# succinctlabs/kzg-rs

Hardware: NVIDIA B200
Metric: blobs verified/sec (verify_blob_kzg_proof_batch) (higher is better)
Workload: dtype u32-limb modular integer (Fr 255-bit / Fp 381-bit) + SHA-256

## Files before the change

### include/kzgb200.h

```cpp
#ifndef KZGB200_H
#define KZGB200_H
#include <stddef.h>
#include <stdint.h>
#ifdef __cplusplus
extern "C" {
#endif

#define KZGB200_OK 0
#define KZGB200_BAD_ARGS 1
#define KZGB200_INTERNAL_ERROR 2
#define KZGB200_INVALID_LENGTH 3
#define KZGB200_INVALID_SETUP 5

#define KZGB200_BYTES_PER_BLOB 131072
#define KZGB200_BYTES_PER_COMMITMENT 48
#define KZGB200_BYTES_PER_PROOF 48
#define KZGB200_BYTES_PER_FIELD_ELEMENT 32
#define KZGB200_PARTIAL_BYTES 352

typedef struct kzgb200_ctx kzgb200_ctx;

int kzgb200_create(kzgb200_ctx** out, int device, const uint8_t* g2_points, size_t g2_points_len);
void kzgb200_destroy(kzgb200_ctx* ctx);
const char* kzgb200_last_error(const kzgb200_ctx* ctx);

int kzgb200_verify_kzg_proof(kzgb200_ctx* ctx, const uint8_t* commitment48, const uint8_t* z32, const uint8_t* y32,
                             const uint8_t* proof48, int* ok);

int kzgb200_verify_blob_kzg_proof(kzgb200_ctx* ctx, const uint8_t* blob, const uint8_t* commitment48,
                                  const uint8_t* proof48, int* ok, uint8_t* z_out, uint8_t* y_out);

int kzgb200_verify_blob_kzg_proof_batch(kzgb200_ctx* ctx, const uint8_t* blobs, size_t n_blobs,
                                        const uint8_t* commitments, size_t n_commitments,
                                        const uint8_t* proofs, size_t n_proofs, int* ok,
                                        uint8_t* z_out, uint8_t* y_out);
int kzgb200_verify_blob_kzg_proof_batch_device(kzgb200_ctx* ctx, const uint8_t* d_blobs, const uint8_t* d_commitments,
                                               const uint8_t* d_proofs, size_t n, int* ok,
                                               uint8_t* d_z_out, uint8_t* d_y_out);

int kzgb200_verify_kzg_proof_many(kzgb200_ctx* ctx, const uint8_t* commitments, const uint8_t* zs, const uint8_t* ys,
                                  const uint8_t* proofs, size_t m, uint8_t* verdicts);

int kzgb200_verify_kzg_proof_batch(kzgb200_ctx* ctx, const uint8_t* commitments104, const uint8_t* zs32, const uint8_t* ys32,
                                   const uint8_t* proofs104, size_t n, int* ok);

int kzgb200_verify_blob_kzg_proof_batch_each(kzgb200_ctx* ctx, const uint8_t* blobs, const uint8_t* commitments, const uint8_t* proofs,
                                             size_t n, uint8_t* verdicts, uint8_t* z_out, uint8_t* y_out);

int kzgb200_compute_challenge(kzgb200_ctx* ctx, const uint8_t* blob, const uint8_t* commitment48, uint8_t* z_out32);
int kzgb200_evaluate_polynomial_in_evaluation_form(kzgb200_ctx* ctx, const uint8_t* blob, const uint8_t* z32, uint8_t* y_out32);

typedef struct kzgb200_group kzgb200_group;
int kzgb200_group_create(kzgb200_group** out, const int* device_ids, int n_devices, const uint8_t* g2_points, size_t g2_points_len,
                         size_t max_blobs_per_device);
int kzgb200_group_join(kzgb200_group** out, const char* session, int rank, int world, int device, const uint8_t* g2_points,
                       size_t g2_points_len, size_t max_blobs_per_rank);
void kzgb200_group_destroy(kzgb200_group* g);
int kzgb200_group_size(const kzgb200_group* g);
int kzgb200_group_local_members(const kzgb200_group* g);
kzgb200_ctx* kzgb200_group_context(kzgb200_group* g, int local_index);
const char* kzgb200_group_last_error(const kzgb200_group* g);
int kzgb200_group_uses_peer_stores(const kzgb200_group* g, int local_index);
int kzgb200_group_verify_blob_kzg_proof_batch(kzgb200_group* g, const uint8_t* blobs, size_t n_blobs, const uint8_t* commitments,
                                              size_t n_commitments, const uint8_t* proofs, size_t n_proofs, int* ok, uint8_t* z_out,
                                              uint8_t* y_out);
int kzgb200_group_verify_shards(kzgb200_group* g, const uint8_t* const* blobs, const uint8_t* const* commitments,
                                const uint8_t* const* proofs, const size_t* n_local, int device_pointers, int* ok,
                                uint8_t* const* z_out, uint8_t* const* y_out);
int kzgb200_group_last_partials(kzgb200_group* g, uint8_t* out, size_t n_ranks);
int kzgb200_group_host_protocol_test(const char* session, int rank, int world, const uint8_t* commitments, const uint8_t* zy,
                                     const uint8_t* proofs, size_t n_local, size_t chunk, uint8_t* digest_out32);

#define KZGB200_TRANSCRIPT_EXACT 0
#define KZGB200_TRANSCRIPT_TREE 1
#define KZGB200_TRANSCRIPT_EXACT_DEVICE 2
int kzgb200_set_transcript_mode(kzgb200_ctx* ctx, int mode);
int kzgb200_last_r(kzgb200_ctx* ctx, uint8_t* r_out32);
int kzgb200_host_sha256(const uint8_t* msg, size_t len, uint8_t* out32, int force_portable);

int kzgb200_last_partial(kzgb200_ctx* ctx, uint8_t* out352);

int kzgb200_harness_generate(kzgb200_ctx* ctx, uint64_t seed, size_t n, int degree, const uint8_t* tau_powers48,
                             uint8_t* d_blobs, uint8_t* d_commitments, uint8_t* d_proofs);
int kzgb200_load_g1_lagrange(kzgb200_ctx* ctx, const uint8_t* g1_lagrange, size_t n_points);
int kzgb200_blob_to_kzg_commitment_batch(kzgb200_ctx* ctx, const uint8_t* d_blobs, size_t n, uint8_t* d_commitments_out);
int kzgb200_compute_blob_kzg_proof_batch(kzgb200_ctx* ctx, const uint8_t* d_blobs, const uint8_t* d_commitments, size_t n,
                                         uint8_t* d_proofs_out);

int kzgb200_load_cell_setup(kzgb200_ctx* ctx, const uint8_t* g1_monomial48, size_t n_points, const uint8_t* g2_tau64_96);
int kzgb200_verify_cell_kzg_proof_batch(kzgb200_ctx* ctx, const uint8_t* commitments, const uint64_t* cell_indices, const uint8_t* cells,
                                        const uint8_t* proofs, size_t n, int* ok);
int kzgb200_verify_cell_kzg_proof_batch_device(kzgb200_ctx* ctx, const uint8_t* d_commitments, const uint64_t* d_cell_indices,
                                               const uint8_t* d_cells, const uint8_t* d_proofs, size_t n, int* ok);
int kzgb200_compute_cells(kzgb200_ctx* ctx, const uint8_t* blob, uint8_t* cells_out);
int kzgb200_compute_cells_batch_device(kzgb200_ctx* ctx, const uint8_t* d_blobs, size_t n, uint8_t* d_cells);
int kzgb200_harness_generate_cells(kzgb200_ctx* ctx, uint64_t seed, size_t n_blobs, int degree, const uint8_t* tau_powers48,
                                   uint8_t* d_cells, uint8_t* d_commitments, uint8_t* d_proofs);

int kzgb200_set_profiling(kzgb200_ctx* ctx, int on);
int kzgb200_set_slab_tail(kzgb200_ctx* ctx, int on);
int kzgb200_get_phase_ms(kzgb200_ctx* ctx, float* out8);
int kzgb200_debug_final_ticks(kzgb200_ctx* ctx, long long* out14);
int kzgb200_debug_engine_selftest(kzgb200_ctx* ctx, uint32_t seed, int rounds, uint32_t* mismatches32, int* n_programs);
void* kzgb200_stream(kzgb200_ctx* ctx);

typedef struct kzgb200_pipeline kzgb200_pipeline;
int kzgb200_pipeline_create(kzgb200_pipeline** out, int device, const uint8_t* g2_points, size_t g2_points_len, int depth);
void kzgb200_pipeline_destroy(kzgb200_pipeline* p);
int kzgb200_pipeline_depth(const kzgb200_pipeline* p);
kzgb200_ctx* kzgb200_pipeline_context(kzgb200_pipeline* p, int slot);
int kzgb200_pipeline_submit(kzgb200_pipeline* p, const uint8_t* blobs, size_t n_blobs, const uint8_t* commitments,
                            size_t n_commitments, const uint8_t* proofs, size_t n_proofs, uint8_t* z_out, uint8_t* y_out,
                            uint64_t* ticket);
int kzgb200_pipeline_submit_device(kzgb200_pipeline* p, const uint8_t* d_blobs, const uint8_t* d_commitments,
                                   const uint8_t* d_proofs, size_t n, uint8_t* d_z_out, uint8_t* d_y_out, uint64_t* ticket);
int kzgb200_pipeline_wait(kzgb200_pipeline* p, uint64_t ticket, int* ok);

void* kzgb200_alloc_pinned(size_t bytes);
void kzgb200_free_pinned(void* p);

#ifdef __cplusplus
}
#endif
#endif
```

### kzg_rs_b200/csrc/common.cuh

```cuda
#pragma once
#include <cuda_runtime.h>
#include "sha256.cuh"
#include "verify.cuh"
#include "vliw.cuh"
#include "vliw29.cuh"
#include "glv.cuh"

namespace kzgb200 {

constexpr int kFieldElementsPerBlob = 4096;
constexpr int kBytesPerBlob = 4096 * 32;
constexpr uint32_t kErrBlob = 1, kErrCommitment = 2, kErrProof = 4, kErrScalar = 8;
struct ZY { Fr z, y; };

struct DeviceTables {
    Fr twiddle[2048];
    Fr twiddle_po[128][32];
    PairingTables pairing;
    vliw29::LineCoeffs29 lines29[2][kMillerSteps];
    G1Affine gen_table[64][15];
    uint32_t setup_ok;
};

#ifndef KSHA_THREADS
// ... 32 lines not shown
}
__device__ __forceinline__ Fr ldg_fr(const Fr* p) {
    const uint4* q = reinterpret_cast<const uint4*>(p);
    uint4 a = __ldg(q), b = __ldg(q + 1);
    Fr f;
    f.l[0] = a.x; f.l[1] = a.y; f.l[2] = a.z; f.l[3] = a.w; f.l[4] = b.x; f.l[5] = b.y; f.l[6] = b.z; f.l[7] = b.w;
    return f;
}

struct Partial {
    G1 a, b;
    Fr ry;
    uint32_t err;
    uint32_t pad[7];
};

struct FinalSmem {
    G1 sm[kFinalThreads];
    unsigned char pad[20 * 1024];
};
struct PairSmem {
    f29::F29 regs[vliw29::kTotalRegs];
    vliw29::SharedTables stab;
};
struct FinalPts { G1Affine pts[2]; uint32_t go; };

constexpr int kManyStride = vliw::kTotalRegsThr * 12 + 1;
constexpr int kManySmemBytes = kManyGroups * kManyStride * 4 + (int)sizeof(vliw::SharedTables) + vliw::kNumSharedRegs * (int)sizeof(Fp) +
                               kManyGroups * (2 * (int)sizeof(G1Affine) + 2) + 64;
struct CellTables {
    Fr w4096[2048], w4096_inv[2048];
    Fr coset[4096];
    Fr shift64[kCellsPerExtBlob];
    Fr shift_inv[kCellsPerExtBlob];
    Fr w64_inv[kFieldElementsPerCell / 2];
    Fr omega8192, inv64;
    G1Affine tau_tab[kFieldElementsPerCell][4];
    LineCoeffs tau64_lines[kMillerSteps];
    vliw29::LineCoeffs29 lines29[kMillerSteps];
    uint32_t ok;
};
__global__ void setup_tables_kernel(DeviceTables* T, const uint8_t* g2_points);
__global__ void setup_lines29_kernel(DeviceTables* T);
constexpr int kChallengeSlabs = 8;
void launch_challenge(int stages, cudaStream_t st, const uint8_t* blobs, const uint8_t* commitments, int n, Fr* z_mont, ZY* zy, Fr* zpow,
                      const uint8_t* slab_flags = nullptr);
__global__ void eval_kernel(const uint8_t* __restrict__ blobs, int n, const Fr* __restrict__ zpow, const DeviceTables* __restrict__ T,
                            ZY* __restrict__ zy, uint32_t* __restrict__ status);
__global__ void g1_decompress_kernel(const uint8_t* __restrict__ commitments, const uint8_t* __restrict__ proofs, int n, G1Affine* __restrict__ C,
                                     G1Affine* __restrict__ P, uint32_t* __restrict__ status, bool with_subgroup_check);
__global__ void g1_subgroup_kernel(const G1Affine* __restrict__ C, const G1Affine* __restrict__ P, int n, uint32_t* __restrict__ status);
__global__ void transcript_schedule_kernel(const uint8_t* __restrict__ commitments, const ZY* __restrict__ zy, const uint8_t* __restrict__ proofs,
                                           uint64_t n, uint32_t* __restrict__ wk, uint64_t first_blk, uint64_t blk_count);
__global__ void transcript_chain_kernel(const uint32_t* __restrict__ wk_all, uint64_t n, Fr* __restrict__ r_mont, uint32_t* __restrict__ state,
                                        uint64_t first_blk, uint64_t blk_count);
__global__ void transcript_words_kernel(const uint8_t* __restrict__ commitments, const ZY* __restrict__ zy, const uint8_t* __restrict__ proofs,
                                        uint64_t first_entry, uint64_t entry_count, uint32_t* __restrict__ words);
__global__ void transcript_tree_leaf_words_kernel(const uint32_t* __restrict__ words, uint64_t n, uint32_t* __restrict__ digests,
                                                  uint64_t first_group, uint64_t group_count);
__global__ void r_from_digest_kernel(const uint32_t* __restrict__ digest, Fr* __restrict__ r_mont);
__global__ void z_setup_kernel(const uint8_t* __restrict__ z_be32, int n, Fr* __restrict__ z_mont, ZY* __restrict__ zy, Fr* __restrict__ zpow,
                               uint32_t* __restrict__ status);
__global__ void import_parsed_kernel(const uint8_t* __restrict__ c104, const uint8_t* __restrict__ p104, const uint8_t* __restrict__ z32,
                                     const uint8_t* __restrict__ y32, int n, G1Affine* __restrict__ C, G1Affine* __restrict__ P,
                                     uint8_t* __restrict__ c48, uint8_t* __restrict__ p48, Fr* __restrict__ z_mont, ZY* __restrict__ zy);
__global__ void msm_scalars_kernel(const Fr* __restrict__ z_mont, const ZY* __restrict__ zy, const Fr* __restrict__ r_mont, uint64_t offset, int n,
                                   uint8_t* __restrict__ digits, Fr* __restrict__ ry);
__global__ void msm_sort_kernel(const uint8_t* __restrict__ digits, int n, uint32_t* __restrict__ order, uint32_t* __restrict__ start);
void launch_msm_bucket(int ctas_per_sm, int n, int slice, cudaStream_t st, const G1Affine* C, const G1Affine* P, const uint32_t* order,
                       const uint32_t* start, G1* halfsum, G1* part);
void launch_msm_bucket_join(int lanes, int n, int slice, cudaStream_t st, const uint32_t* start, const G1* halfsum, const G1* part, G1* buckets);
__global__ void msm_window_kernel(const G1* __restrict__ buckets, G1* __restrict__ windows);
__global__ void msm_combine_kernel(const G1* __restrict__ windows, const Fr* __restrict__ ry, const uint32_t* __restrict__ status, int n,
                                   const DeviceTables* __restrict__ T, Partial* __restrict__ out, uint32_t* flag, uint32_t epoch);
__global__ void wait_flags_kernel(const uint32_t* flags, int count, uint32_t epoch, uint32_t* __restrict__ timed_out);
__global__ void batch_final_kernel(const Partial* __restrict__ parts, int nparts, const DeviceTables* __restrict__ T, uint32_t* __restrict__ result,
                                   FinalPts* __restrict__ out);
__global__ void single_final_kernel(const G1Affine* __restrict__ C, const G1Affine* __restrict__ P, const ZY* __restrict__ zy,
                                    const uint32_t* __restrict__ status, const DeviceTables* __restrict__ T, uint32_t* __restrict__ result,
                                    FinalPts* __restrict__ out);
__global__ void pairing_check_kernel(const FinalPts* __restrict__ in, const DeviceTables* __restrict__ T, const vliw29::LineCoeffs29* __restrict__ lines_b,
                                     uint32_t* __restrict__ result, long long* __restrict__ ticks);
__global__ void engine_selftest_kernel(uint32_t seed, int rounds, f29::F29* __restrict__ ref, uint32_t* __restrict__ mismatches);
inline void launch_batch_final(cudaStream_t st, const Partial* parts, int nparts, const DeviceTables* T, uint32_t* result, unsigned char* scratch512,
                               bool ticks, const vliw29::LineCoeffs29* lines_b = nullptr) {
    FinalPts* fp = reinterpret_cast<FinalPts*>(scratch512 + 256);
    batch_final_kernel<<<1, kFinalThreads, sizeof(FinalSmem), st>>>(parts, nparts, T, result, fp);
    pairing_check_kernel<<<1, kPairThreads, sizeof(PairSmem), st>>>(fp, T, lines_b, result, ticks ? reinterpret_cast<long long*>(scratch512 + 128) : nullptr);
}
__global__ void many_lhs_kernel(const uint8_t* __restrict__ z32, const uint8_t* __restrict__ y32, const G1Affine* __restrict__ C,
                                const G1Affine* __restrict__ P, size_t m, const DeviceTables* __restrict__ T, G1Affine* __restrict__ X,
                                uint32_t* __restrict__ status);
__global__ void many_lhs_zy_kernel(const ZY* __restrict__ zy, const G1Affine* __restrict__ C, const G1Affine* __restrict__ P, size_t m,
                                   const DeviceTables* __restrict__ T, G1Affine* __restrict__ X, const uint32_t* __restrict__ status);
__global__ void many_pairing_kernel(const G1Affine* __restrict__ X, const G1Affine* __restrict__ P, const uint32_t* __restrict__ status, size_t m,
                                    const DeviceTables* __restrict__ T, uint8_t* __restrict__ verdicts);
__global__ void many_pairing_warp_kernel(const G1Affine* __restrict__ X, const G1Affine* __restrict__ P, size_t m, const DeviceTables* __restrict__ T,
                                         uint8_t* __restrict__ verdicts);
__global__ void export_scalars_kernel(const ZY* __restrict__ zy, int n, uint8_t* __restrict__ z_out, uint8_t* __restrict__ y_out);
__global__ void r_to_raw_kernel(const Fr* __restrict__ r_mont, ZY* __restrict__ out);
__global__ void status_or_kernel(const uint32_t* __restrict__ status, int n, uint32_t* __restrict__ out);
__global__ void harness_parse_points_kernel(const uint8_t* bytes, int n, G1Affine* out, uint32_t* bad);
__global__ void harness_blob_kernel(uint64_t seed, int n, int D, const DeviceTables* __restrict__ T, uint8_t* __restrict__ blobs);
__global__ void harness_commit_kernel(uint64_t seed, int n, int D, const G1Affine* __restrict__ M, const Fr* __restrict__ z_mont,
                                      uint8_t* __restrict__ out, int want_proof);
__global__ void lag_parse_kernel(const uint8_t* __restrict__ bytes, G1Affine* __restrict__ out, uint32_t* __restrict__ bad);
__global__ void lag_table_kernel(const G1Affine* __restrict__ L, G1* __restrict__ table);
__global__ void blob_scalars_kernel(const uint8_t* __restrict__ blobs, int n, Fr* __restrict__ scalars, uint32_t* __restrict__ status);
__global__ void quotient_kernel(const uint8_t* __restrict__ blobs, int n, const Fr* __restrict__ z_mont, const ZY* __restrict__ zy,
                                const DeviceTables* __restrict__ T, Fr* __restrict__ scalars);
__global__ void lag_msm_kernel(const Fr* __restrict__ scalars, int n, const G1* __restrict__ table, uint8_t* __restrict__ out48);
__global__ void cell_setup_kernel(CellTables* T, const uint8_t* __restrict__ g2_tau64);
__global__ void cell_setup_points_kernel(CellTables* T, const uint8_t* __restrict__ g1_monomial48);
__global__ void cell_setup_lines29_kernel(CellTables* T);
__global__ void compute_cells_kernel(const uint8_t* __restrict__ blobs, int n, const CellTables* __restrict__ T, uint8_t* __restrict__ cells,
                                     uint32_t* __restrict__ status);
__global__ void cell_points_kernel(const uint8_t* __restrict__ bytes, int count, G1Affine* __restrict__ out, uint32_t* __restrict__ status, uint32_t flag);
__global__ void cell_check_kernel(const uint8_t* __restrict__ cells, int n, uint32_t* __restrict__ status);
__global__ void cell_scalars_kernel(const uint32_t* __restrict__ meta, int n, const G1Affine* __restrict__ U, const uint32_t* __restrict__ ustatus,
                                    const CellTables* __restrict__ T, Fr* __restrict__ z_mont, ZY* __restrict__ zy, G1Affine* __restrict__ C,
                                    uint32_t* __restrict__ status);
__global__ void cell_rpow_kernel(const Fr* __restrict__ r_mont, int n, Fr* __restrict__ rk);
__global__ void cell_agg_kernel(const uint8_t* __restrict__ cells, const uint32_t* __restrict__ meta, int n, const Fr* __restrict__ rk, Fr* __restrict__ agg);
__global__ void cell_interp_kernel(const Fr* __restrict__ agg, const uint32_t* __restrict__ meta, int n, const CellTables* __restrict__ T,
                                   Fr* __restrict__ coeffs);
__global__ void cell_rli_kernel(const Fr* __restrict__ coeffs, const CellTables* __restrict__ T, Partial* __restrict__ out);
__global__ void cell_harness_terms_kernel(uint64_t seed, int n, int D, const G1Affine* __restrict__ M, G1* __restrict__ terms);
__global__ void cell_harness_sums_kernel(int n, const G1* __restrict__ terms, G1* __restrict__ sums);
__global__ void cell_harness_points_kernel(int n, const G1* __restrict__ sums, const CellTables* __restrict__ T, uint8_t* __restrict__ commitments,
                                           uint8_t* __restrict__ proofs);
__global__ void cell_harness_eval_kernel(uint64_t seed, int n, int D, const CellTables* __restrict__ T, uint8_t* __restrict__ cells);

}
```

### kzg_rs_b200/csrc/k_final.cu

```cuda
#include "common.cuh"
#include "coop.cuh"

namespace kzgb200 {

__global__ void __launch_bounds__(kFinalThreads) batch_final_kernel(const Partial* __restrict__ parts, int nparts, const DeviceTables* __restrict__ T,
                                                                    uint32_t* __restrict__ result, FinalPts* __restrict__ out) {
    extern __shared__ __align__(16) unsigned char dyn_smem[];
    FinalSmem& S = *reinterpret_cast<FinalSmem*>(dyn_smem);
    G1* sm = S.sm;
    __shared__ Fr s_sum;
    __shared__ uint32_t s_err;
    int t = threadIdx.x;
    if (t == 0) result[2] = 0;
    if (t == 0) {
        Fr s = Fr::zero(); uint32_t err = 0;
        for (int k = 0; k < nparts; k++) { s = s.add_inl(parts[k].ry); err |= parts[k].err; }
        s_sum = s; s_err = err;
    }
    __syncthreads();
    if (s_err) { if (t == 0) { result[0] = kBadArgs; result[1] = s_err; out->go = 0; } return; }
    G1 sg = G1::identity();
    if (!s_sum.is_zero()) sg = coop_fixed_base_mul(s_sum, T, sm);
    if ((t & 31) == 0) {
        int w = t >> 5;
        G1 acc = G1::identity();
        for (int k = 0; k < nparts; k++) acc = acc.add(w == 0 ? parts[k].a : parts[k].b);
        if (w == 1) acc = acc.add(sg.neg());
        Fp zi = vliw::fp_inv_bingcd(acc.z), zi2 = zi.sqr();
        G1Affine a = acc.is_identity() ? G1Affine{Fp::zero(), Fp::zero(), 1} : G1Affine{acc.x * zi2, acc.y * zi2 * zi, 0};
        if (w == 0 && !a.inf) a.y = a.y.neg();
        out->pts[w] = a;
        if (w == 0) out->go = 1;
    }
}

__global__ void __launch_bounds__(kPairThreads) pairing_check_kernel(const FinalPts* __restrict__ in, const DeviceTables* __restrict__ T,
                                                                     const vliw29::LineCoeffs29* __restrict__ lines_b, uint32_t* __restrict__ result,
                                                                     long long* __restrict__ ticks) {
    extern __shared__ __align__(16) unsigned char dyn_smem[];
    PairSmem& S = *reinterpret_cast<PairSmem*>(dyn_smem);
    const int t = threadIdx.x;
    if (in->go == 0) return;
    if (ticks && t == 0) { ticks[0] = clock64(); for (int i = 6; i < 14; i++) ticks[i] = 0; }
    vliw29::Tables tab = vliw29::load_tables(&S.stab, t, kPairThreads);
    vliw29::Lanes L{t, kPairThreads, tab, ticks, S.stab.p29};
    const G1Affine p0 = in->pts[0], p1 = in->pts[1];
    bool ok = vliw29::coop_pairing_product_is_one(S.regs, p1, T->lines29[0], p0, lines_b ? lines_b : T->lines29[1], L);
    L.tick(5);
    if (t == 0) { result[0] = ok ? kTrue : kFalse; result[1] = 0; }
}

__global__ void __launch_bounds__(kPairThreads) engine_selftest_kernel(uint32_t seed, int rounds, f29::F29* __restrict__ ref, uint32_t* __restrict__ mismatches) {
    extern __shared__ __align__(16) unsigned char dyn_smem[];
    PairSmem& S = *reinterpret_cast<PairSmem*>(dyn_smem);
    const int t = threadIdx.x;
    vliw29::Tables tab = vliw29::load_tables(&S.stab, t, kPairThreads);
    vliw29::Lanes L{t, kPairThreads, tab, nullptr, S.stab.p29};
    for (int i = t; i < vliw29::kTotalRegs; i += kPairThreads) {
        Fp x;
        uint32_t s = seed * 2654435761u + (uint32_t)i * 40503u + 1u;
        for (int k = 0; k < 12; k++) { s = s * 1664525u + 1013904223u; x.l[k] = s; }
        x.l[11] &= 0x0fffffffu;
        f29::F29 v = f29::from_fp(x);
        if (i >= vliw29::kRegConst && i < vliw29::kRegConst + 10) v = vliw29::frob_const(i - vliw29::kRegConst);
        S.regs[i] = v; ref[i] = v;
    }
    __syncthreads();
    for (int r = 0; r < rounds; r++)
        for (int prog = 0; prog < vliw29::kNumPrograms; prog++) {
            vliw29::run(prog, S.regs, L);
            if (t == 32) vliw29::run_ref(prog, ref, vliw29::default_tables());
            __syncthreads();
            for (int i = t; i < vliw29::kTotalRegs; i += kPairThreads)
                if (!(vliw29::canonical_signed(S.regs[i], 2048) == vliw29::canonical_signed(ref[i], 2048))) atomicAdd(&mismatches[prog], 1u);
            __syncthreads();
        }
}

}
```

### kzg_rs_b200/csrc/kzgb200.cu

```cuda
#include <new>
#include "runtime.cuh"

using namespace kzgb200;

namespace kzgb200 {
CopyPool::CopyPool(int nthreads) {
    for (int i = 0; i < nthreads; i++) threads.emplace_back([this] {
        uint64_t seen = 0;
        for (;;) {
            {
                std::unique_lock<std::mutex> lk(m);
                cv.wait(lk, [&] { return stop || gen != seen; });
                if (stop) return;
                seen = gen;
            }
            work(seen);
        }
    });
}
CopyPool::~CopyPool() {
    { std::lock_guard<std::mutex> lk(m); stop = true; }
    cv.notify_all();
    for (auto& t : threads) t.join();
}
// ... 799 lines not shown
    CK(cudaMalloc(&ctx->d_lag_table, (size_t)kFieldElementsPerBlob * kLagWindows * kLagEntries * sizeof(G1)));
    CK(cudaMemsetAsync(d_bad, 0, 4, ctx->stream));
    CK(cudaMemcpyAsync(d_bytes, g1_lagrange, n_points * 48, cudaMemcpyHostToDevice, ctx->stream));
    lag_parse_kernel<<<(kFieldElementsPerBlob + 127) / 128, 128, 0, ctx->stream>>>(d_bytes, d_L, d_bad);
    lag_table_kernel<<<(kFieldElementsPerBlob * kLagWindows + 127) / 128, 128, 0, ctx->stream>>>(d_L, ctx->d_lag_table);
    CK(cudaGetLastError());
    CK(cudaMemcpyAsync(&bad, d_bad, 4, cudaMemcpyDeviceToHost, ctx->stream));
    CK(cudaStreamSynchronize(ctx->stream));
    cudaFree(d_bytes); cudaFree(d_L); cudaFree(d_bad);
    if (bad) { cudaFree(ctx->d_lag_table); ctx->d_lag_table = nullptr; return KZGB200_INVALID_SETUP; }
    return KZGB200_OK;
}
static int commit_or_prove(kzgb200_ctx* ctx, const uint8_t* d_blobs, const uint8_t* d_commitments, size_t n, uint8_t* d_out, int want_proof) {
    if (!ctx->d_lag_table) return KZGB200_INVALID_SETUP;
    const size_t kChunk = 1024;
    int rc = ensure_capacity(ctx, n < kChunk ? n : kChunk, false);
    if (rc) return rc;
    if (!ctx->d_scalars) CK(cudaMalloc(&ctx->d_scalars, kChunk * (size_t)kFieldElementsPerBlob * sizeof(Fr)));
    uint32_t any_bad = 0;
    for (size_t lo = 0; lo < n; lo += kChunk) {
        int cnt = (int)(n - lo < kChunk ? n - lo : kChunk);
        const uint8_t* blobs = d_blobs + lo * kBytesPerBlob;
        CK(cudaMemsetAsync(ctx->d_status, 0, cnt * sizeof(uint32_t), ctx->stream));
        if (!want_proof) {
            blob_scalars_kernel<<<(unsigned)(((size_t)cnt * kFieldElementsPerBlob + 127) / 128), 128, 0, ctx->stream>>>(blobs, cnt, ctx->d_scalars, ctx->d_status);
        } else {
            launch_challenge(ctx->sha_stages, ctx->stream, blobs, d_commitments + lo * 48, cnt, ctx->d_z_mont, ctx->d_zy, ctx->d_zpow);
            eval_kernel<<<cnt, kEvalThreads, 0, ctx->stream>>>(blobs, cnt, ctx->d_zpow, ctx->tables, ctx->d_zy, ctx->d_status);
            quotient_kernel<<<cnt, kEvalThreads, 0, ctx->stream>>>(blobs, cnt, ctx->d_z_mont, ctx->d_zy, ctx->tables, ctx->d_scalars);
        }
        lag_msm_kernel<<<cnt, 256, 0, ctx->stream>>>(ctx->d_scalars, cnt, ctx->d_lag_table, d_out + lo * 48);
        status_or_kernel<<<1, 256, 0, ctx->stream>>>(ctx->d_status, cnt, ctx->d_result);
        CK(cudaGetLastError());
        CK(cudaMemcpyAsync(ctx->h_result, ctx->d_result, 4, cudaMemcpyDeviceToHost, ctx->stream));
        CK(cudaStreamSynchronize(ctx->stream));
        any_bad |= ctx->h_result[0];
    }
    return any_bad ? KZGB200_BAD_ARGS : KZGB200_OK;
}
extern "C" int kzgb200_blob_to_kzg_commitment_batch(kzgb200_ctx* ctx, const uint8_t* d_blobs, size_t n, uint8_t* d_commitments_out) {
    if (!ctx || !d_blobs || !d_commitments_out || n == 0) return KZGB200_BAD_ARGS;
    std::lock_guard<std::mutex> g(ctx->lock);
    DeviceGuard dev(ctx->device);
    return commit_or_prove(ctx, d_blobs, nullptr, n, d_commitments_out, 0);
}
extern "C" int kzgb200_compute_blob_kzg_proof_batch(kzgb200_ctx* ctx, const uint8_t* d_blobs, const uint8_t* d_commitments, size_t n,
                                                    uint8_t* d_proofs_out) {
    if (!ctx || !d_blobs || !d_commitments || !d_proofs_out || n == 0) return KZGB200_BAD_ARGS;
    std::lock_guard<std::mutex> g(ctx->lock);
    DeviceGuard dev(ctx->device);
    return commit_or_prove(ctx, d_blobs, d_commitments, n, d_proofs_out, 1);
}
extern "C" int kzgb200_debug_final_ticks(kzgb200_ctx* ctx, long long* out14) {
    if (!ctx || !out14) return KZGB200_BAD_ARGS;
    std::lock_guard<std::mutex> g(ctx->lock);
    DeviceGuard dev(ctx->device);
    CK(cudaMemcpy(out14, ctx->d_scratch + 128, 112, cudaMemcpyDeviceToHost));
    return KZGB200_OK;
}
extern "C" int kzgb200_set_slab_tail(kzgb200_ctx* ctx, int on) {
    if (!ctx) return KZGB200_BAD_ARGS;
    std::lock_guard<std::mutex> g(ctx->lock);
    ctx->slab_tail = on != 0;
    return KZGB200_OK;
}
extern "C" int kzgb200_debug_engine_selftest(kzgb200_ctx* ctx, uint32_t seed, int rounds, uint32_t* mismatches32, int* n_programs) {
    if (!ctx || !mismatches32 || !n_programs || rounds < 1) return KZGB200_BAD_ARGS;
    std::lock_guard<std::mutex> g(ctx->lock);
    DeviceGuard dev(ctx->device);
    f29::F29* d_ref = nullptr; uint32_t* d_mis = nullptr;
    CK(cudaMalloc(&d_ref, sizeof(f29::F29) * vliw29::kTotalRegs));
    CK(cudaMalloc(&d_mis, 32 * sizeof(uint32_t)));
    CK(cudaMemsetAsync(d_mis, 0, 32 * sizeof(uint32_t), ctx->stream));
    CK(cudaFuncSetAttribute(engine_selftest_kernel, cudaFuncAttributeMaxDynamicSharedMemorySize, (int)sizeof(PairSmem)));
    engine_selftest_kernel<<<1, kPairThreads, sizeof(PairSmem), ctx->stream>>>(seed, rounds, d_ref, d_mis);
    CK(cudaGetLastError());
    CK(cudaMemcpyAsync(mismatches32, d_mis, 32 * sizeof(uint32_t), cudaMemcpyDeviceToHost, ctx->stream));
    CK(cudaStreamSynchronize(ctx->stream));
    cudaFree(d_ref); cudaFree(d_mis);
    *n_programs = vliw29::kNumPrograms;
    static_assert(vliw29::kNumPrograms <= 32, "mismatch array");
    return KZGB200_OK;
}
extern "C" void* kzgb200_stream(kzgb200_ctx* ctx) { return ctx ? (void*)ctx->stream : nullptr; }

extern "C" void* kzgb200_alloc_pinned(size_t bytes) {
    void* p = nullptr;
    return cudaMallocHost(&p, bytes) == cudaSuccess ? p : nullptr;
}
extern "C" void kzgb200_free_pinned(void* p) { if (p) cudaFreeHost(p); }

static void cell_destroy(kzgb200_ctx* ctx) {
    CellCtx* c = ctx->cells;
    if (!c) return;
    void* d[] = {c->tables, c->d_cells, c->d_p, c->d_uc, c->d_meta, c->d_ustatus, c->d_U, c->d_rk, c->d_agg, c->d_coeffs, c->d_part, c->d_ext};
    for (void* p : d) if (p) cudaFree(p);
    void* h[] = {c->h_meta, c->h_uc, c->h_c, c->h_cells, c->h_p, c->h_idx};
    for (void* p : h) if (p) cudaFreeHost(p);
    for (cudaEvent_t e : {c->ev_r, c->ev_rli}) if (e) cudaEventDestroy(e);
    delete c;
    ctx->cells = nullptr;
}

extern "C" int kzgb200_load_cell_setup(kzgb200_ctx* ctx, const uint8_t* g1_monomial48, size_t n_points, const uint8_t* g2_tau64_96) {
    if (!ctx) return KZGB200_BAD_ARGS;
    if (!g1_monomial48 || n_points < (size_t)kFieldElementsPerCell || !g2_tau64_96) return KZGB200_INVALID_SETUP;
    std::lock_guard<std::mutex> g(ctx->lock);
    DeviceGuard dev(ctx->device);
    if (ctx->cells) return KZGB200_OK;
    CellCtx* c = new (std::nothrow) CellCtx();
    if (!c) return KZGB200_INTERNAL_ERROR;
    ctx->cells = c;
    uint8_t* d_bytes = nullptr;
    uint32_t ok = 0;
    int rc = [&]() -> int {
        CK(cudaMalloc(&c->tables, sizeof(CellTables)));
        CK(cudaMalloc(&d_bytes, kFieldElementsPerCell * 48 + 96));
        CK(cudaMemcpyAsync(d_bytes, g1_monomial48, kFieldElementsPerCell * 48, cudaMemcpyHostToDevice, ctx->stream));
        CK(cudaMemcpyAsync(d_bytes + kFieldElementsPerCell * 48, g2_tau64_96, 96, cudaMemcpyHostToDevice, ctx->stream));
        cell_setup_kernel<<<4096 / 128, 128, 0, ctx->stream>>>(c->tables, d_bytes + kFieldElementsPerCell * 48);
        cell_setup_points_kernel<<<kFieldElementsPerCell * 4 / 64, 64, 0, ctx->stream>>>(c->tables, d_bytes);
        cell_setup_lines29_kernel<<<(kMillerSteps * 6 + 127) / 128, 128, 0, ctx->stream>>>(c->tables);
        CK(cudaGetLastError());
        CK(cudaMemcpyAsync(&ok, &c->tables->ok, 4, cudaMemcpyDeviceToHost, ctx->stream));
        CK(cudaStreamSynchronize(ctx->stream));
        CK(cudaFuncSetAttribute(compute_cells_kernel, cudaFuncAttributeMaxDynamicSharedMemorySize, kCellNttSmemBytes));
        CK(cudaMalloc(&c->d_agg, (size_t)kCellsPerExtBlob * kCellAggSlices * kFieldElementsPerCell * sizeof(Fr)));
        CK(cudaMalloc(&c->d_coeffs, (size_t)kCellsPerExtBlob * kFieldElementsPerCell * sizeof(Fr)));
        CK(cudaMalloc(&c->d_part, 2 * sizeof(Partial)));
        CK(cudaEventCreateWithFlags(&c->ev_r, cudaEventDisableTiming));
        CK(cudaEventCreateWithFlags(&c->ev_rli, cudaEventDisableTiming));
        return KZGB200_OK;
    }();
    if (d_bytes) cudaFree(d_bytes);
    if (rc == KZGB200_OK && !ok) rc = KZGB200_INVALID_SETUP;
    if (rc != KZGB200_OK) cell_destroy(ctx);
    return rc;
}

static int cell_capacity(kzgb200_ctx* ctx, size_t n, bool host_inputs, bool device_inputs) {
    CellCtx* c = ctx->cells;
    int rc = ensure_capacity(ctx, n, false);
    if (rc) return rc;
    if (n > c->cap) {
        CK(regrow(c->d_meta, 3 * n + kCellsPerExtBlob + 1)); CK(regrow(c->d_ustatus, n)); CK(regrow(c->d_uc, n * 48));
        CK(regrow(c->d_U, n)); CK(regrow(c->d_rk, n));
        if (c->d_cells) { cudaFree(c->d_cells); c->d_cells = nullptr; }
        if (c->d_p) { cudaFree(c->d_p); c->d_p = nullptr; }
        c->cap = n;
        c->slot.assign(1, 0);
    }
    if (host_inputs && !c->d_cells) { CK(cudaMalloc(&c->d_cells, c->cap * kBytesPerCell)); CK(cudaMalloc(&c->d_p, c->cap * 48)); }
    if (n > c->host_cap) {
        for (void* p : {(void*)c->h_meta, (void*)c->h_uc, (void*)c->h_c, (void*)c->h_cells, (void*)c->h_p, (void*)c->h_idx}) if (p) cudaFreeHost(p);
        c->h_meta = nullptr; c->h_uc = c->h_c = c->h_cells = c->h_p = nullptr; c->h_idx = nullptr;
        CK(cudaMallocHost(&c->h_meta, (3 * n + kCellsPerExtBlob + 1) * 4)); CK(cudaMallocHost(&c->h_uc, n * 48));
        c->host_cap = n;
    }
    if (device_inputs && !c->h_cells) {
        CK(cudaMallocHost(&c->h_c, c->host_cap * 48)); CK(cudaMallocHost(&c->h_cells, c->host_cap * kBytesPerCell));
        CK(cudaMallocHost(&c->h_p, c->host_cap * 48)); CK(cudaMallocHost(&c->h_idx, c->host_cap * 8));
    }
    return KZGB200_OK;
}

static size_t cell_plan(CellCtx* c, const uint8_t* commitments, const uint64_t* idx, size_t n) {
// ... 204 lines not shown
```

### kzg_rs_b200/csrc/vliw29.cuh

```cuda
#pragma once
#include "vliw.cuh"
#include "fp29.cuh"
#include "vliw29_programs.cuh"

namespace kzgb200 {
namespace vliw29 {
using f29::F29;
constexpr int32_t kM = (int32_t)f29::kMask;

struct Tables {
    const uint32_t (*mul)[4];
    const uint32_t (*lin)[4];
    const uint32_t* term;
    const Level* level;
    const Program* prog;
};
constexpr int kGroupLanes = 16;
struct Lanes {
    int tid, n;
    Tables tab;
    long long* ticks = nullptr;
    const int32_t* p29s = nullptr;
    int groups = 1, gstride = 0;
    int bar_id = 0, bar_threads = 0;
// ... 38 lines not shown
}
#endif

#define KZG29_FROB_TABLE {KZG29_FROB6_1_C0, KZG29_FROB6_1_C1, KZG29_FROB6_2_C0, KZG29_FROB6_2_C1, KZG29_FROB6_3_C0, KZG29_FROB6_3_C1, \
                          KZG29_FROB6_4_C0, KZG29_FROB6_4_C1, KZG29_FROB6_5_C0, KZG29_FROB6_5_C1}
#ifdef __CUDACC__
static __device__ const uint32_t d_frob29[10][14] = KZG29_FROB_TABLE;
#endif
KZG_HD F29 frob_const(int i) {
    F29 r;
#ifdef __CUDA_ARCH__
    for (int k = 0; k < 14; k++) r.l[k] = d_frob29[i][k];
#else
    static const uint32_t h[10][14] = KZG29_FROB_TABLE;
    for (int k = 0; k < 14; k++) r.l[k] = h[i][k];
#endif
    r.l[14] = r.l[15] = 0;
    return r;
}

KZG_HD void normalize_ref(F29& r, int64_t* t) {
    for (int i = 0; i < 13; i++) { r.l[i] = (uint32_t)t[i] & f29::kMask; t[i + 1] += t[i] >> 29; }
    r.l[13] = (uint32_t)t[13]; r.l[14] = 0; r.l[15] = 0;
}
KZG_HD int32_t limb(const F29& v, int i) { return (int32_t)v.l[i]; }
KZG_NI void exec_mul_ref(F29* regs, const uint32_t* ins) {
    const uint32_t w0 = ins[0], w1 = ins[1], w2 = ins[2];
    const bool dual = (w2 >> 16) & 1u, neg = (w2 >> 17) & 1u;
    const F29 a = regs[w0 >> 16], b = regs[w1 & 0xffffu];
    int64_t t[29];
    for (int k = 0; k < 29; k++) t[k] = 0;
    for (int i = 0; i < 14; i++) for (int j = 0; j < 14; j++) t[i + j] += (int64_t)limb(a, i) * limb(b, j);
    if (dual) {
        const F29 c = regs[w1 >> 16], d = regs[w2 & 0xffffu];
        for (int i = 0; i < 14; i++) for (int j = 0; j < 14; j++) t[i + j] += (int64_t)(neg ? -limb(c, i) : limb(c, i)) * limb(d, j);
    }
    for (int k = 0; k < 28; k++) { int64_t c = t[k] >> 29; t[k] &= f29::kMask; t[k + 1] += c; }
    for (int i = 0; i < 14; i++) {
        int64_t m = (int64_t)(((uint32_t)t[i] * KZG29_PINV) & f29::kMask);
        for (int j = 0; j < 14; j++) t[i + j] += m * (int64_t)f29::p29_rt(j);
        t[i + 1] += t[i] >> 29;
    }
    t[27] += t[28] << 29;
    F29 r;
    normalize_ref(r, t + 14);
    regs[w0 & 0xffffu] = r;
}
KZG_NI void exec_lin_ref(F29* regs, const uint32_t* ins, const uint32_t* terms) {
    int64_t t[14];
    for (int i = 0; i < 14; i++) t[i] = 0;
    for (uint32_t k = 0; k < ins[2]; k++) {
        const uint32_t e = terms[ins[1] + k];
        const F29& v = regs[(e & 0xffffu) >> 6];
        const int32_t coef = (int32_t)e >> 16;
        for (int i = 0; i < 14; i++) t[i] += (int64_t)limb(v, i) * coef;
    }
    if (ins[3] & 1u) {
        const float vf = (float)t[13] * 536870912.0f + (float)t[12];
        const float pinv = 1.0f / ((float)f29::p29_rt(13) * 536870912.0f + (float)f29::p29_rt(12));
        const int32_t q = (int32_t)rintf(vf * pinv);
        for (int i = 0; i < 14; i++) t[i] -= (int64_t)f29::p29_rt(i) * q;
    }
    F29 r;
    normalize_ref(r, t);
    regs[ins[0]] = r;
}

#ifdef __CUDACC__
constexpr unsigned kFull = 0xffffffffu;
__device__ __forceinline__ int32_t up(int32_t v, int d, int lane) { int32_t r = __shfl_up_sync(kFull, v, d, kGroupLanes); return lane < d ? 0 : r; }
__device__ __forceinline__ int32_t from(int32_t v, int src) { return __shfl_sync(kFull, v, src, kGroupLanes); }
__device__ __forceinline__ int32_t carry_top(int64_t t, int lane) {
    const bool top = lane >= 13;
    const int64_t c64 = t >> 29;
    int32_t low = top ? (int32_t)t : ((int32_t)t & kM);
    int32_t cmid = top ? 0 : (lane == 12 ? (int32_t)c64 : ((int32_t)c64 & kM));
    int32_t chi = (top || lane == 12) ? 0 : (int32_t)(t >> 58);
    int32_t l = low + up(cmid, 1, lane) + up(chi, 2, lane);
    int32_t c = top ? 0 : (l >> 29);
    l = top ? l : (l & kM);
    return l + up(c, 1, lane);
}
__device__ __forceinline__ int64_t mulw(int32_t a, int32_t b) { uint64_t r = 0; f29::madw_s(r, a, b); return (int64_t)r; }
__device__ __forceinline__ int32_t up32(int32_t v, int d, int k) { int32_t r = __shfl_up_sync(kFull, v, d); return k < d ? 0 : r; }
__device__ __forceinline__ int32_t rot(int32_t v, int k, int s) { return __shfl_sync(kFull, v, (k - s) & 31); }
__device__ __forceinline__ int32_t carry_split(int64_t& t, int k, int nlow) {
    const bool lowlane = k < nlow;
    const int32_t low = lowlane ? ((int32_t)t & kM) : 0, cmid = lowlane ? ((int32_t)(t >> 29) & kM) : 0, chi = lowlane ? (int32_t)(t >> 58) : 0;
    const int32_t u1 = up32(cmid, 1, k), u2 = up32(chi, 2, k);
    int32_t l = low + u1 + u2;
    if (!lowlane) t += (int64_t)u1 + (int64_t)u2;
    const int32_t c = lowlane ? (l >> 29) : 0;
    const int32_t u = up32(c, 1, k);
    l = lowlane ? ((l & kM) + u) : 0;
    if (!lowlane) t += (int64_t)u;
    return l;
}
__device__ __forceinline__ int32_t carry_full(int64_t t, int k) {
    const bool top = k >= 27;
    const int64_t c64 = t >> 29;
    const int32_t low = top ? (int32_t)t : ((int32_t)t & kM);
    const int32_t cmid = top ? 0 : (k == 26 ? (int32_t)c64 : ((int32_t)c64 & kM));
    const int32_t chi = (top || k == 26) ? 0 : (int32_t)(t >> 58);
    int32_t l = low + up32(cmid, 1, k) + up32(chi, 2, k);
    const int32_t c = top ? 0 : (l >> 29);
    l = top ? l : (l & kM);
    return l + up32(c, 1, k);
}
__device__ __forceinline__ void exec_mul32(F29* regs, const uint32_t* ins, int k) {
    const uint32_t w0 = ins[0], w1 = ins[1], w2 = ins[2];
    const bool dual = (w2 >> 16) & 1u, neg = (w2 >> 17) & 1u;
    uint64_t acc = 0, acc1 = 0;
    {
        const int32_t av = k < 16 ? reinterpret_cast<const int32_t*>(regs[w0 >> 16].l)[k] : 0;
        const int4* B = reinterpret_cast<const int4*>(regs[w1 & 0xffffu].l);
        const int4 b0 = B[0], b1 = B[1], b2 = B[2], b3 = B[3];
        const int32_t bb[14] = {b0.x, b0.y, b0.z, b0.w, b1.x, b1.y, b1.z, b1.w, b2.x, b2.y, b2.z, b2.w, b3.x, b3.y};
#pragma unroll
        for (int s = 0; s < 14; s++) f29::madw_s((s & 1) ? acc1 : acc, rot(av, k, s), bb[s]);
    }
    if (dual) {
        int32_t cv = k < 16 ? reinterpret_cast<const int32_t*>(regs[w1 >> 16].l)[k] : 0;
        if (neg) cv = -cv;
        const int4* D = reinterpret_cast<const int4*>(regs[w2 & 0xffffu].l);
        const int4 d0 = D[0], d1 = D[1], d2 = D[2], d3 = D[3];
        const int32_t dd[14] = {d0.x, d0.y, d0.z, d0.w, d1.x, d1.y, d1.z, d1.w, d2.x, d2.y, d2.z, d2.w, d3.x, d3.y};
#pragma unroll
        for (int s = 0; s < 14; s++) f29::madw_s((s & 1) ? acc1 : acc, rot(cv, k, s), dd[s]);
    }
    int64_t hi = (int64_t)(acc + acc1);
    const int32_t tl = carry_split(hi, k, 14);
    uint64_t mc = 0, mc1 = 0;
    {
        constexpr uint32_t pinv[14] = KZG29_PINV_FULL;
#pragma unroll
        for (int s = 0; s < 14; s++) f29::madw_s((s & 1) ? mc1 : mc, rot(tl, k, s), (int32_t)pinv[s]);
    }
    int64_t mcol = k < 14 ? (int64_t)(mc + mc1) : 0;
    int32_t m = carry_split(mcol, k, 14);
    if (k == 13) m &= kM;
    uint64_t mp = 0, mp1 = 0;
    {
        constexpr uint32_t pp[14] = KZG29_P;
#pragma unroll
        for (int s = 0; s < 14; s++) f29::madw_s((s & 1) ? mp1 : mp, rot(m, k, s), (int32_t)pp[s]);
    }
    const int64_t tot = (k < 14 ? (int64_t)tl : hi) + (int64_t)(mp + mp1);
    int32_t r = carry_full(tot, k);
    const int32_t z13 = __shfl_sync(kFull, r, 13);
    if (k == 14) r += (z13 + (1 << 28)) >> 29;
    if (k >= 14 && k < 30) reinterpret_cast<int32_t*>(regs[w0 & 0xffffu].l)[k - 14] = k < 28 ? r : 0;
}
__device__ __forceinline__ void exec_lin16(F29* regs, const uint32_t* ins, const uint32_t* terms, bool active, const int32_t* p29s, int lane) {
    int32_t sl = 0, sh = 0;
    const uint32_t* tt = terms + ins[1];
    const uint32_t count = ins[2];
    const unsigned char* base = reinterpret_cast<const unsigned char*>(regs) + 4 * lane;
#pragma unroll 4
    for (uint32_t k = 0; k < count; k++) {
        const uint32_t e = tt[k];
        const int32_t v = *reinterpret_cast<const int32_t*>(base + (e & 0xffffu));
        const int32_t coef = (int32_t)e >> 16;
        sl += (v & 0xffff) * coef;
        sh += (v >> 16) * coef;
    }
    int64_t t = (int64_t)sl + ((int64_t)sh << 16);
    if (__any_sync(kFull, ins[3] & 1u)) {
        const float f = lane == 13 ? (float)t * 536870912.0f : (lane == 12 ? (float)t : 0.0f);
        const float vf = __shfl_sync(kFull, f, 13, kGroupLanes) + __shfl_sync(kFull, f, 12, kGroupLanes);
        if (ins[3] & 1u) {
            const float pinv = 1.0f / ((float)f29::p29_rt(13) * 536870912.0f + (float)f29::p29_rt(12));
            const int32_t q = (int32_t)rintf(vf * pinv);
            t -= mulw(p29s[lane], q);
        }
    }
    const int32_t r = carry_top(t, lane);
    if (active) reinterpret_cast<int32_t*>(regs[ins[0]].l)[lane] = r;
}
#endif

KZG_HD void run(int prog, F29* regs, const Lanes& L) {
    const Program p = L.tab.prog[prog];
    for (int lv = p.first_level; lv < p.first_level + p.n_levels; lv++) {
        const Level lev = L.tab.level[lv];
#ifdef __CUDA_ARCH__
        long long c0 = L.ticks ? clock64() : 0;
        const int total = lev.count * L.groups;
        if (lev.kind == 1) {
            const int w = L.tid >> 5, nw = L.n >> 5;
            const int passes = (total + nw - 1) / nw, per = (total + passes - 1) / passes;
            if (w < per)
                for (int i = w; i < total; i += per) {
                    const int k = L.groups == 1 ? i : i / L.groups, g = i - k * L.groups;
                    exec_mul32(regs + g * L.gstride, L.tab.mul[lev.first + k], L.tid & 31);
                }
        } else {
            const int slot = L.tid >> 4, nslots = L.n >> 4, lane = L.tid & 15;
            for (int base = 0; base < total; base += nslots) {
                const int i = base + slot;
                if (base + (slot & ~1) >= total) break;
                const bool active = i < total;
                const int ii = active ? i : base, k = L.groups == 1 ? ii : ii / L.groups, g = ii - k * L.groups;
                exec_lin16(regs + g * L.gstride, L.tab.lin[lev.first + k], L.tab.term, active, L.p29s, lane);
            }
        }
        long long c1 = L.ticks ? clock64() : 0;
#else
        for (int g = 0; g < L.groups; g++) {
            if (lev.kind == 1) { for (int k = 0; k < lev.count; k++) exec_mul_ref(regs + g * L.gstride, L.tab.mul[lev.first + k]); }
            else { for (int k = 0; k < lev.count; k++) exec_lin_ref(regs + g * L.gstride, L.tab.lin[lev.first + k], L.tab.term); }
        }
#endif
        L.sync();
#ifdef __CUDA_ARCH__
        if (L.ticks && L.tid == 0) {
            long long c2 = clock64();
            int b = lev.kind == 1 ? 10 : 8;
            L.ticks[b] += c1 - c0; L.ticks[b + 1] += c2 - c1; L.ticks[b == 10 ? 13 : 12] += 1;
        }
#endif
    }
}
KZG_NI void run_ref(int prog, F29* regs, const Tables& tab) {
    const Program p = tab.prog[prog];
    for (int lv = p.first_level; lv < p.first_level + p.n_levels; lv++) {
        const Level lev = tab.level[lv];
        if (lev.kind == 1) { for (int k = 0; k < lev.count; k++) exec_mul_ref(regs, tab.mul[lev.first + k]); }
        else { for (int k = 0; k < lev.count; k++) exec_lin_ref(regs, tab.lin[lev.first + k], tab.term); }
    }
}
KZG_HD void copy_regs(F29* regs, int dst, int src, int count, const Lanes& L) {
    uint4* d = reinterpret_cast<uint4*>(regs + dst);
    const uint4* s = reinterpret_cast<const uint4*>(regs + src);
    for (int j = L.tid; j < count * 4; j += L.n) d[j] = s[j];
    L.sync();
}

struct LineCoeffs29 { F29 v[6]; };
KZG_HD void load_lines(F29* regs, const LineCoeffs29* c1, const LineCoeffs29* c2, int k, const Lanes& L) {
    uint4* d = reinterpret_cast<uint4*>(regs + kRegLines);
    for (int q = L.tid; q < 2 * 6 * 4; q += L.n) {
        const LineCoeffs29* src = q < 24 ? c1 : c2;
        if (!src) continue;
        d[q] = reinterpret_cast<const uint4*>(src[k].v)[q < 24 ? q : q - 24];
    }
    L.sync();
}

KZG_NI Fp canonical_signed(const F29& v, int bound = kIoBound) {
    int64_t t[14];
    for (int i = 0; i < 14; i++) t[i] = (int64_t)limb(v, i) + (int64_t)bound * (int64_t)f29::p29_rt(i);
    F29 u;
    normalize_ref(u, t);
    return f29::canonical(u);
}
KZG_NI F29 inv29(const F29& v) {
    Fp x = canonical_signed(v), y;
    vliw::fp_inv_raw(y.l, x.l);
    return f29::from_raw(y);
}

constexpr int kSave0 = kMaxRegs;
constexpr int kNumSaves = 5;
constexpr int kTotalRegs = kMaxRegs + 12 * kNumSaves;

KZG_HD bool coop_pairing_product_is_one(F29* regs, const G1Affine& P1, const LineCoeffs29* c1, const G1Affine& P2, const LineCoeffs29* c2,
                                        const Lanes& L) {
    const bool live1 = !P1.inf, live2 = !P2.inf;
    if (!live1 && !live2) return true;
    const G1Affine& Pa = live1 ? P1 : P2;
    const LineCoeffs29* ca = live1 ? c1 : c2;
    const LineCoeffs29* cb = (live1 && live2) ? c2 : nullptr;
    for (int i = L.tid; i < 26; i += L.n) {
        if (i < 10) regs[kRegConst + i] = frob_const(i);
        else if (i < 14) {
            const int j = i - 10;
            if (j < 2) regs[kRegP + j] = f29::from_fp(j == 0 ? Pa.x : Pa.y);
            else regs[kRegP + j] = cb ? f29::from_fp(j == 2 ? P2.x : P2.y) : f29::f29_zero();
        } else regs[kRegF + (i - 14)] = i == 14 ? f29::f29_one() : f29::f29_zero();
// ... 41 lines not shown
```

Before: 1.597 million.

## Run two Montgomery multiplies per warp using half-warp lanes when level is wide

```diff
diff --git a/include/kzgb200.h b/include/kzgb200.h
--- a/include/kzgb200.h
+++ b/include/kzgb200.h
@@ -102,6 +102,7 @@
 int kzgb200_get_phase_ms(kzgb200_ctx* ctx, float* out8);
 int kzgb200_debug_final_ticks(kzgb200_ctx* ctx, long long* out14);
 int kzgb200_debug_engine_selftest(kzgb200_ctx* ctx, uint32_t seed, int rounds, uint32_t* mismatches32, int* n_programs);
+int kzgb200_debug_engine_mul(kzgb200_ctx* ctx, uint32_t* regs, int nregs, const uint32_t* rows, int count, uint32_t* ref);
 void* kzgb200_stream(kzgb200_ctx* ctx);
 
 typedef struct kzgb200_pipeline kzgb200_pipeline;
diff --git a/kzg_rs_b200/csrc/common.cuh b/kzg_rs_b200/csrc/common.cuh
--- a/kzg_rs_b200/csrc/common.cuh
+++ b/kzg_rs_b200/csrc/common.cuh
@@ -138,6 +138,7 @@
 __global__ void pairing_check_kernel(const FinalPts* __restrict__ in, const DeviceTables* __restrict__ T, const vliw29::LineCoeffs29* __restrict__ lines_b,
                                      uint32_t* __restrict__ result, long long* __restrict__ ticks);
 __global__ void engine_selftest_kernel(uint32_t seed, int rounds, f29::F29* __restrict__ ref, uint32_t* __restrict__ mismatches);
+__global__ void engine_mul_kernel(f29::F29* __restrict__ regs, int nregs, const uint32_t* __restrict__ rows, int count, f29::F29* __restrict__ ref);
 inline void launch_batch_final(cudaStream_t st, const Partial* parts, int nparts, const DeviceTables* T, uint32_t* result, unsigned char* scratch512,
                                bool ticks, const vliw29::LineCoeffs29* lines_b = nullptr) {
     FinalPts* fp = reinterpret_cast<FinalPts*>(scratch512 + 256);
diff --git a/kzg_rs_b200/csrc/k_final.cu b/kzg_rs_b200/csrc/k_final.cu
--- a/kzg_rs_b200/csrc/k_final.cu
+++ b/kzg_rs_b200/csrc/k_final.cu
@@ -77,4 +77,19 @@
         }
 }
 
+__global__ void __launch_bounds__(kPairThreads) engine_mul_kernel(f29::F29* __restrict__ regs, int nregs, const uint32_t* __restrict__ rows, int count,
+                                                                  f29::F29* __restrict__ ref) {
+    extern __shared__ __align__(16) unsigned char dyn_smem[];
+    PairSmem& S = *reinterpret_cast<PairSmem*>(dyn_smem);
+    const int t = threadIdx.x;
+    vliw29::Lanes L{t, kPairThreads, vliw29::default_tables(), nullptr, nullptr};
+    for (int i = t; i < nregs; i += kPairThreads) { S.regs[i] = regs[i]; ref[i] = regs[i]; }
+    __syncthreads();
+    vliw29::run_mul_level(S.regs, reinterpret_cast<const uint32_t (*)[4]>(rows), count, L);
+    if (t == 32)
+        for (int k = 0; k < count; k++) vliw29::exec_mul_ref(ref, rows + 4 * k);
+    __syncthreads();
+    for (int i = t; i < nregs; i += kPairThreads) regs[i] = S.regs[i];
 }
+
+}
diff --git a/kzg_rs_b200/csrc/kzgb200.cu b/kzg_rs_b200/csrc/kzgb200.cu
--- a/kzg_rs_b200/csrc/kzgb200.cu
+++ b/kzg_rs_b200/csrc/kzgb200.cu
@@ -905,6 +905,33 @@
     static_assert(vliw29::kNumPrograms <= 32, "mismatch array");
     return KZGB200_OK;
 }
+extern "C" int kzgb200_debug_engine_mul(kzgb200_ctx* ctx, uint32_t* regs, int nregs, const uint32_t* rows, int count, uint32_t* ref) {
+    if (!ctx || !regs || !rows || !ref || nregs < 1 || nregs > vliw29::kTotalRegs || count < 1 || count > 1024) return KZGB200_BAD_ARGS;
+    for (int k = 0; k < count; k++) {
+        const uint32_t* r = rows + 4 * k;
+        const bool dual = (r[2] >> 16) & 1u;
+        const uint32_t ids[5] = {r[0] & 0xffffu, r[0] >> 16, r[1] & 0xffffu, dual ? r[1] >> 16 : 0u, dual ? r[2] & 0xffffu : 0u};
+        for (uint32_t id : ids)
+            if (id >= (uint32_t)nregs) return KZGB200_BAD_ARGS;
+    }
+    std::lock_guard<std::mutex> g(ctx->lock);
+    DeviceGuard dev(ctx->device);
+    const size_t bytes = sizeof(f29::F29) * nregs;
+    f29::F29 *d_regs = nullptr, *d_ref = nullptr; uint32_t* d_rows = nullptr;
+    CK(cudaMalloc(&d_regs, bytes));
+    CK(cudaMalloc(&d_ref, bytes));
+    CK(cudaMalloc(&d_rows, 16 * (size_t)count));
+    CK(cudaMemcpyAsync(d_regs, regs, bytes, cudaMemcpyHostToDevice, ctx->stream));
+    CK(cudaMemcpyAsync(d_rows, rows, 16 * (size_t)count, cudaMemcpyHostToDevice, ctx->stream));
+    CK(cudaFuncSetAttribute(engine_mul_kernel, cudaFuncAttributeMaxDynamicSharedMemorySize, (int)sizeof(PairSmem)));
+    engine_mul_kernel<<<1, kPairThreads, sizeof(PairSmem), ctx->stream>>>(d_regs, nregs, d_rows, count, d_ref);
+    CK(cudaGetLastError());
+    CK(cudaMemcpyAsync(regs, d_regs, bytes, cudaMemcpyDeviceToHost, ctx->stream));
+    CK(cudaMemcpyAsync(ref, d_ref, bytes, cudaMemcpyDeviceToHost, ctx->stream));
+    CK(cudaStreamSynchronize(ctx->stream));
+    cudaFree(d_regs); cudaFree(d_ref); cudaFree(d_rows);
+    return KZGB200_OK;
+}
 extern "C" void* kzgb200_stream(kzgb200_ctx* ctx) { return ctx ? (void*)ctx->stream : nullptr; }
 
 extern "C" void* kzgb200_alloc_pinned(size_t bytes) {
diff --git a/kzg_rs_b200/csrc/vliw29.cuh b/kzg_rs_b200/csrc/vliw29.cuh
--- a/kzg_rs_b200/csrc/vliw29.cuh
+++ b/kzg_rs_b200/csrc/vliw29.cuh
@@ -144,8 +144,87 @@
     return l + up(c, 1, lane);
 }
 __device__ __forceinline__ int64_t mulw(int32_t a, int32_t b) { uint64_t r = 0; f29::madw_s(r, a, b); return (int64_t)r; }
+template <class B>
+__device__ __forceinline__ void mul_rows(uint64_t& c0, uint64_t& c1, int32_t x0, int32_t y0, int j, B b) {
+    int32_t x = x0, y = y0;
+#pragma unroll
+    for (int s = 0; s < 14; s++) {
+        f29::madw_s(c0, x, b(s));
+        f29::madw_s(c1, y, b(s));
+        if (s < 13) {
+            const int32_t nx = (s & 1) ? __shfl_sync(kFull, x0, j - (s + 1) / 2, kGroupLanes) : __shfl_sync(kFull, y0, j - s / 2 - 1, kGroupLanes);
+            y = x;
+            x = nx;
+        }
+    }
+}
+__device__ __forceinline__ void carry_low(int64_t& t0, int64_t& t1, int32_t& l0, int32_t& l1, int j) {
+    const bool low = j < 7;
+    if (low) { t1 += t0 >> 29; t0 &= kM; }
+    const int32_t rm = up(low ? ((int32_t)(t1 >> 29) & kM) : 0, 1, j), rh = up(low ? (int32_t)(t1 >> 58) : 0, 1, j);
+    t0 += rm;
+    t1 = (low ? (t1 & kM) : t1) + rh;
+    l0 = (int32_t)t0; l1 = (int32_t)t1;
+    l1 += l0 >> 29; l0 &= kM;
+    const int32_t c = low ? (l1 >> 29) : 0;
+    l1 &= kM;
+    const int32_t rc = up(c, 1, j);
+    l0 += rc;
+    if (!low) { t0 += rc; l0 = 0; l1 = 0; }
+}
+__device__ __forceinline__ void exec_mul_pair(F29* regs, const uint32_t* ins, int j, bool active) {
+    const uint32_t w0 = ins[0], w1 = ins[1], w2 = ins[2];
+    const bool dual = (w2 >> 16) & 1u, neg = (w2 >> 17) & 1u;
+    uint64_t acc0 = 0, acc1 = 0;
+    {
+        const int2 av = j < 8 ? reinterpret_cast<const int2*>(regs[w0 >> 16].l)[j] : make_int2(0, 0);
+        const int4* B = reinterpret_cast<const int4*>(regs[w1 & 0xffffu].l);
+        const int4 b0 = B[0], b1 = B[1], b2 = B[2], b3 = B[3];
+        const int32_t bb[14] = {b0.x, b0.y, b0.z, b0.w, b1.x, b1.y, b1.z, b1.w, b2.x, b2.y, b2.z, b2.w, b3.x, b3.y};
+        mul_rows(acc0, acc1, av.x, av.y, j, [&](int s) { return bb[s]; });
+    }
+    if (__any_sync(kFull, dual)) {
+        int2 cv = dual && j < 8 ? reinterpret_cast<const int2*>(regs[w1 >> 16].l)[j] : make_int2(0, 0);
+        if (neg) { cv.x = -cv.x; cv.y = -cv.y; }
+        const int4* D = reinterpret_cast<const int4*>(regs[(dual ? w2 : w1) & 0xffffu].l);
+        const int4 d0 = D[0], d1 = D[1], d2 = D[2], d3 = D[3];
+        const int32_t dd[14] = {d0.x, d0.y, d0.z, d0.w, d1.x, d1.y, d1.z, d1.w, d2.x, d2.y, d2.z, d2.w, d3.x, d3.y};
+        mul_rows(acc0, acc1, cv.x, cv.y, j, [&](int s) { return dd[s]; });
+    }
+    int64_t h0 = (int64_t)acc0, h1 = (int64_t)acc1;
+    int32_t tl0, tl1;
+    carry_low(h0, h1, tl0, tl1, j);
+    uint64_t mc0 = 0, mc1 = 0;
+    {
+        constexpr uint32_t pinv[14] = KZG29_PINV_FULL;
+        mul_rows(mc0, mc1, tl0, tl1, j, [&](int s) { return (int32_t)pinv[s]; });
+    }
+    int64_t m0 = (int64_t)mc0, m1 = (int64_t)mc1;
+    int32_t ml0, ml1;
+    carry_low(m0, m1, ml0, ml1, j);
+    if (j == 6) ml1 &= kM;
+    uint64_t mp0 = 0, mp1 = 0;
+    {
+        constexpr uint32_t pp[14] = KZG29_P;
+        mul_rows(mp0, mp1, ml0, ml1, j, [&](int s) { return (int32_t)pp[s]; });
+    }
+    const bool low = j < 7, top = j >= 13;
+    int64_t u0 = (low ? (int64_t)tl0 : h0) + (int64_t)mp0, u1 = (low ? (int64_t)tl1 : h1) + (int64_t)mp1;
+    u1 += u0 >> 29; u0 &= kM;
+    const int32_t rm = up(top ? 0 : ((int32_t)(u1 >> 29) & kM), 1, j), rh = up(top ? 0 : (int32_t)(u1 >> 58), 1, j);
+    u0 += rm;
+    u1 = (top ? u1 : (u1 & kM)) + rh;
+    const int32_t z13 = __shfl_sync(kFull, (int32_t)u1, 6, kGroupLanes);
+    if (j == 7) u0 += (z13 + (1 << 28)) >> 29;
+    int32_t l0 = (int32_t)u0, l1 = (int32_t)u1;
+    l1 += l0 >> 29; l0 &= kM;
+    const int32_t c = (low || top) ? 0 : (l1 >> 29);
+    if (!top) l1 &= kM;
+    l0 += up(c, 1, j);
+    if (active && j >= 7 && j < 15) reinterpret_cast<int2*>(regs[w0 & 0xffffu].l)[j - 7] = j < 14 ? make_int2(l0, l1) : make_int2(0, 0);
+}
 __device__ __forceinline__ int32_t up32(int32_t v, int d, int k) { int32_t r = __shfl_up_sync(kFull, v, d); return k < d ? 0 : r; }
-__device__ __forceinline__ int32_t rot(int32_t v, int k, int s) { return __shfl_sync(kFull, v, (k - s) & 31); }
+__device__ __forceinline__ int32_t rot(int32_t v, int k, int s) { return __shfl_sync(kFull, v, k - s); }
 __device__ __forceinline__ int32_t carry_split(int64_t& t, int k, int nlow) {
     const bool lowlane = k < nlow;
     const int32_t low = lowlane ? ((int32_t)t & kM) : 0, cmid = lowlane ? ((int32_t)(t >> 29) & kM) : 0, chi = lowlane ? (int32_t)(t >> 58) : 0;
@@ -241,22 +320,39 @@
 }
 #endif
 
+#ifdef __CUDACC__
+__device__ __forceinline__ void run_mul_level(F29* regs, const uint32_t (*rows)[4], int count, const Lanes& L) {
+    const int total = count * L.groups;
+    const int w = L.tid >> 5, nw = L.n >> 5, h = (L.tid >> 4) & 1;
+    if (total <= nw) {
+        if (w < total) {
+            const int k = L.groups == 1 ? w : w / L.groups, g = w - k * L.groups;
+            exec_mul32(regs + g * L.gstride, rows[k], L.tid & 31);
+        }
+        return;
+    }
+    const int pairs = (total + 1) >> 1;
+    const int passes = (pairs + nw - 1) / nw, per = (pairs + passes - 1) / passes;
+    if (w >= per) return;
+    for (int q = w; q < pairs; q += per) {
+        const int i = 2 * q + h;
+        const bool active = i < total;
+        const int ii = active ? i : i - 1, k = L.groups == 1 ? ii : ii / L.groups, g = ii - k * L.groups;
+        exec_mul_pair(regs + g * L.gstride, rows[k], L.tid & 15, active);
+    }
+}
+#endif
+
 KZG_HD void run(int prog, F29* regs, const Lanes& L) {
     const Program p = L.tab.prog[prog];
     for (int lv = p.first_level; lv < p.first_level + p.n_levels; lv++) {
         const Level lev = L.tab.level[lv];
 #ifdef __CUDA_ARCH__
         long long c0 = L.ticks ? clock64() : 0;
-        const int total = lev.count * L.groups;
         if (lev.kind == 1) {
-            const int w = L.tid >> 5, nw = L.n >> 5;
-            const int passes = (total + nw - 1) / nw, per = (total + passes - 1) / passes;
-            if (w < per)
-                for (int i = w; i < total; i += per) {
-                    const int k = L.groups == 1 ? i : i / L.groups, g = i - k * L.groups;
-                    exec_mul32(regs + g * L.gstride, L.tab.mul[lev.first + k], L.tid & 31);
-                }
+            run_mul_level(regs, L.tab.mul + lev.first, lev.count, L);
         } else {
+            const int total = lev.count * L.groups;
             const int slot = L.tid >> 4, nslots = L.n >> 4, lane = L.tid & 15;
             for (int base = 0; base < total; base += nslots) {
                 const int i = base + slot;
```

After: 1.626 million, median of 6. +1.8%, better.
